# zzzxxxttt/SimpleDepthEstimation

Hardware: AMD Instinct MI355X
Metric: training images/sec at 192x640 bs=12/GPU (higher is better)
Workload: dtype bf16; 1 GPU; Supervised ResNet-50 (BASELINE configs[1]), bf16 storage / fp32 accumulate, bs=12/GPU, 192x640, fwd+bwd+optimizer, random-init weights; global_batch=12, parallelism=dp1, hip_graph=True, allreduce_overlap=False

## Files before the change

### include/sde_hip.h

```cpp
#ifndef SDE_HIP_H
#define SDE_HIP_H
#include <stddef.h>
#include <stdint.h>

#ifdef __cplusplus
extern "C" {
#endif

typedef void* sde_stream_t;

#define SDE_MAX_CTX 4
#define SDE_F32 0
#define SDE_BF16 1
#define SDE_F16 2

#define SDE_REDUCE_ROWS 32

#define SDE_RESIZE_BILINEAR_AC 0
#define SDE_RESIZE_NEAREST 1

const char* sde_last_error(void);
int sde_version(void);

int sde_mark_time(uint64_t* slot, sde_stream_t stream);
// ... 105 lines not shown
size_t sde_conv_fwd_ws_bytes(const sde_conv_desc* d, int ldy);
int sde_conv_fwd_ws(const sde_conv_desc* d, const void* w_packed, const float* bias, int act, void* y, int Cout, int ldy, float* stats, void* ws,
                    size_t ws_bytes, sde_stream_t stream);
int sde_conv_dgrad_bnbwd_rows(const sde_conv_desc* d, int Cout, int ldy);
int sde_conv_dgrad_bnbwd(const sde_conv_desc* d, const void* w_packed, void* gm, int Cout, int ldy, const void* bn_y, const float* bnp, float* part,
                         sde_stream_t stream);
int sde_conv_dgrad_bnbwd_res_rows(const sde_conv_desc* d, int Cout, int ldy);
int sde_conv_dgrad_bnbwd_res(const sde_conv_desc* d, const void* w_packed, void* gm, int Cout, int ldy, const void* bn_y, const float* bnp, float* part,
                             const void* res_grad, const void* bn_out, sde_stream_t stream);
int sde_conv_fwd_tiles_m(const sde_conv_desc* d, int ldy);
int sde_conv_fwd_variant(const sde_conv_desc* d, int ldy);
int sde_conv_set_halo_min_blocks(int min_blocks);
#define SDE_OPT_PGEMM 1
#define SDE_OPT_PGEMM_DEPTH 2
#define SDE_OPT_PGEMM_3X3 3
#define SDE_OPT_PGEMM_TILE 4
#define SDE_OPT_SPLITK 5
#define SDE_OPT_WGRAD_BLOCKS 6
#define SDE_OPT_WGRAD_HALO 7
#define SDE_OPT_CONV_SMALL 8
#define SDE_OPT_WGRAD_DMA 9
#define SDE_OPT_BNBWD_FUSE 10
#define SDE_OPT_CU_RESERVE 11
int sde_conv_set_option(int key, int value);

#define SDE_WGRAD_FOLD_ROWS 16
int sde_conv_wgrad_splits(const sde_conv_desc* d, int Cout);
int sde_conv_wgrad(const sde_conv_desc* d, const void* dy, int Cout, int ldd, int Cin_real, float* slab, int splits, float* dw, int accumulate,
                   sde_stream_t stream);

int sde_conv_wgrad_partial(const sde_conv_desc* d, const void* dy, int Cout, int ldd, float* slab, int splits, sde_stream_t stream);
typedef struct sde_wreduce_item {
    const float* slab;
    float* dw;
    int32_t rows , Cout, KHW, Cin_pad, Cin_real;
    int32_t accumulate;
} sde_wreduce_item;
#define SDE_WREDUCE_ACCUMULATE 1
#define SDE_WREDUCE_OHWI 2
int sde_wgrad_reduce_batched(const sde_wreduce_item* items, int n, sde_stream_t stream);

int sde_prep_input(const float* img, const float* mean, const float* std_, int B, int C, int H, int W, int Cpad, int flip, int dtype, void* out,
                   sde_stream_t stream);

int sde_bn_finalize(const float* part, int tiles, int C, long count, const float* gamma, const float* beta, float* running_mean, float* running_var,
                    float momentum, float eps, float* bnp, sde_stream_t stream);
// ... 145 lines not shown
```

### simpledepthestimation_amd/csrc/conv.hip

```cpp
#include <type_traits>

#include "common.h"
#include "sde_hip.h"
#include "conv_common.h"

namespace {
using namespace sdeconv;

template <int I> using IC = std::integral_constant<int, I>;

typedef __attribute__((ext_vector_type(4))) float f32x4;
typedef __attribute__((ext_vector_type(8))) __bf16 bf16x8;
typedef __attribute__((ext_vector_type(4))) short s16x4;
typedef __attribute__((ext_vector_type(8))) short s16x8;

template <typename T> struct VecOf;
template <> struct VecOf<float> { static constexpr int V = 4; };
template <> struct VecOf<bf16_t> { static constexpr int V = 8; };
template <> struct VecOf<half_t> { static constexpr int V = 8; };

template <typename T>
__device__ __forceinline__ uint4 gather16(const Gather& g, int n, int ih, int iw, int ci) {
    uint4 z = {0u, 0u, 0u, 0u};
    if (g.reflect) { ih = reflect1(ih, g.IH); iw = reflect1(iw, g.IW); }
// ... 1274 lines not shown
    if (d->src_mode == SDE_SRC_UPCAT) {
        if (d->IH != 2 * d->H0 || d->IW != 2 * d->W0 || (d->C1 > 0 && !d->x1)) { sde_set_error("%s: upcat shape mismatch", who); return SDE_ERR_ARG; }
    } else if (d->src_mode == SDE_SRC_PLAIN) {
        if (d->IH != d->H0 || d->IW != d->W0 || d->C1 != 0) { sde_set_error("%s: plain source shape mismatch", who); return SDE_ERR_ARG; }
    } else if (d->src_mode == SDE_SRC_ZEROINS) {
        if (d->IH > 2 * d->H0 || d->IW > 2 * d->W0 || d->IH < 2 * d->H0 - 1 || d->IW < 2 * d->W0 - 1 || d->C1 != 0) { sde_set_error("%s: zero-insert shape mismatch", who); return SDE_ERR_ARG; }
    } else { sde_set_error("%s: bad src_mode %d", who, d->src_mode); return SDE_ERR_ARG; }
    if (d->reflect && (d->pad >= d->IH || d->pad >= d->IW || d->pad > 1)) { sde_set_error("%s: reflection pad must be 1 and < size", who); return SDE_ERR_ARG; }
    const int oh_max = (d->OH - 1) * d->stride - d->pad + d->KH - 1, ow_max = (d->OW - 1) * d->stride - d->pad + d->KW - 1;
    if (d->reflect && (oh_max > d->IH || ow_max > d->IW)) { sde_set_error("%s: output extent exceeds reflected input", who); return SDE_ERR_ARG; }
    g.x0 = d->x0; g.x1 = d->x1; g.C0 = d->C0; g.C1 = d->C1; g.Cin = d->C0 + d->C1; g.H0 = d->H0; g.W0 = d->W0; g.IH = d->IH; g.IW = d->IW;
    g.mode = d->src_mode; g.KH = d->KH; g.KW = d->KW; g.stride = d->stride; g.pad = d->pad; g.reflect = d->reflect;
    g.Bn = d->Bn; g.OH = d->OH; g.OW = d->OW; g.M = d->Bn * d->OH * d->OW; g.Ktot = d->KH * d->KW * g.Cin;
    if ((long)d->Bn * d->OH * d->OW > 0x7fffffffL) { sde_set_error("%s: too many output pixels", who); return SDE_ERR_ARG; }
    return SDE_OK;
}

}

namespace sdeconv {
bool pgemm_applicable(const Gather& g, int dtype, int ldy);
bool pgemm_bnbwd_ok(const Gather& g, int dtype, int ldy, int Cout, int depth);
int pgemm_tile(const Gather& g, int ldy);
int pgemm_run(const IGemmP& p, int dtype, int depth, hipStream_t s);
int pgemm_stats_rows(const Gather& g, int ldy, int depth, bool bnbwd = false);
bool chalo_applicable(const Gather& g, int dtype, int ldy);
int chalo_run(const IGemmP& p, int dtype, hipStream_t s);
bool wgrad_dma_applicable(const Gather& g, int dtype, int Cout, int ldd);
int wgrad_dma_run(const Gather& g, int dtype, const void* dy, int Cout, int ldd, float* slab, int splits, int rows_per_split, hipStream_t s);
bool whalo_applicable(const Gather& g, int dtype, int Cout, int ldd);
int whalo_splits(const Gather& g, int Cout);
int whalo_run(const Gather& g, int dtype, const void* dy, int Cout, int ldd, float* slab, int splits, hipStream_t s);
extern int g_pgemm_force_tile;
}
namespace {
int g_use_pgemm = 1;
int g_pgemm_depth = 3;
int g_pgemm_3x3 = 0;
int g_splitk = 1;
long g_wgrad_blocks = 256;
bool use_pgemm(const Gather& g, int dtype, int ldy) {
    if (!g_use_pgemm || !pgemm_applicable(g, dtype, ldy)) return false;
    return g_pgemm_3x3 || !use_halo(g, dtype, ldy);
}
}

extern "C" {

static int pick_ksplit(const Gather& g, int dtype, int ldy) {
    const bool pg = use_pgemm(g, dtype, ldy);
    if (!g_splitk || ldy % 4) return 1;
    if (pg ? (pgemm_tile(g, ldy) != 64064 || g.mode == SDE_SRC_ZEROINS) : (use_halo(g, dtype, ldy) || pick_tile(g.M, ldy, g.Ktot) != 64064)) return 1;
    const long tiles = (long)sde_cdiv(g.M, 64) * sde_cdiv(ldy, 64);
    const int nk = sde_cdiv(g.Ktot, SDE_IS16(dtype) ? 64 : 32);
    const long tmax = pg ? 256 : 384, target = pg ? 512 : 768;
    if (pg && tiles >= tmax && tiles < 2 * tmax && nk >= (g_splitk >= 2 ? g_splitk : 48)) return 2;
    if (tiles >= tmax || nk < 16) return 1;
    long S = sde_cdiv(target, tiles);
    if (S > 8) S = 8;
    if (S > nk / 8) S = nk / 8;
    return S < 2 ? 1 : (int)S;
}

int g_conv_small = 1;
static bool use_chalo(const Gather& g, int dtype, int ldy) { return g_conv_small && sdeconv::chalo_applicable(g, dtype, ldy); }

static int conv_fwd_impl(const sde_conv_desc* d, const void* w_packed, const float* bias, int act, void* y, int Cout, int ldy, float* stats,
                         float* ws, size_t ws_bytes, sde_stream_t stream) {
    SDE_CHECK_ARG(d && w_packed && y, "sde_conv_fwd: null pointer");
    IGemmP p;
    int rc = fill_gather(d, p.g, "sde_conv_fwd");
    if (rc) return rc;
    SDE_CHECK_ARG(Cout > 0 && ldy >= Cout, "sde_conv_fwd: bad Cout=%d ldy=%d", Cout, ldy);
    SDE_CHECK_ARG(act == SDE_ACT_NONE || act == SDE_ACT_ELU, "sde_conv_fwd: bad act %d", act);
    p.w = w_packed; p.bias = bias; p.y = y; p.stats = stats; p.Cout = Cout; p.ldy = ldy; p.act = act;
    p.ksplit = 1; p.ws = nullptr;
    p.no_kfull = 0;
    p.bn_y = nullptr; p.bnp = nullptr; p.bn_gb = nullptr; p.bn_out = nullptr;
    const int S = ws ? pick_ksplit(p.g, d->dtype, ldy) : 1;
    if (S > 1) {
        SDE_CHECK_ARG(ws_bytes >= (size_t)S * p.g.M * ldy * sizeof(float), "sde_conv_fwd_ws: workspace too small (%zu bytes)", ws_bytes);
        p.ksplit = S; p.ws = ws;
    }
    if (!stats && p.ksplit == 1 && use_chalo(p.g, d->dtype, ldy)) {
        sdeconv::chalo_run(p, d->dtype, (hipStream_t)stream);
    } else if (use_pgemm(p.g, d->dtype, ldy)) {
        SDE_CHECK_ARG((p.ksplit - 1) * sde_cdiv(p.g.Ktot / 64, p.ksplit) < p.g.Ktot / 64, "sde_conv_fwd: empty K split");
        SDE_CHECK_ARG(p.ksplit == 1 || sdeconv::pgemm_stats_rows(p.g, ldy, g_pgemm_depth) == sde_cdiv(p.g.M, 64), "sde_conv_fwd: split-K layer with per-workgroup statistics");
        sdeconv::pgemm_run(p, d->dtype, g_pgemm_depth, (hipStream_t)stream);
    } else if (use_halo(p.g, d->dtype, ldy)) {
        if (d->dtype == SDE_BF16) dispatch_halo<bf16_t>(p, (hipStream_t)stream); else dispatch_halo<half_t>(p, (hipStream_t)stream);
    } else if (d->dtype == SDE_BF16) dispatch_igemm<bf16_t>(p, (hipStream_t)stream);
    else if (d->dtype == SDE_F16) dispatch_igemm<half_t>(p, (hipStream_t)stream);
    else dispatch_igemm<float>(p, (hipStream_t)stream);
    SDE_CHECK_LAUNCH("sde_conv_fwd");
    if (S > 1) {
        const unsigned nb = (unsigned)(sde_cdiv(p.g.M, 64) * sde_cdiv(ldy, 64));
        if (d->dtype == SDE_BF16) hipLaunchKernelGGL(splitk_finish_kernel<bf16_t>, dim3(nb), dim3(256), 0, (hipStream_t)stream, ws, S, p.g.M, ldy, Cout, bias, act, (bf16_t*)y, stats);
        else if (d->dtype == SDE_F16) hipLaunchKernelGGL(splitk_finish_kernel<half_t>, dim3(nb), dim3(256), 0, (hipStream_t)stream, ws, S, p.g.M, ldy, Cout, bias, act, (half_t*)y, stats);
        else hipLaunchKernelGGL(splitk_finish_kernel<float>, dim3(nb), dim3(256), 0, (hipStream_t)stream, ws, S, p.g.M, ldy, Cout, bias, act, (float*)y, stats);
        SDE_CHECK_LAUNCH("sde_conv_fwd/splitk_finish");
    }
    return SDE_OK;
}

int sde_conv_fwd(const sde_conv_desc* d, const void* w_packed, const float* bias, int act, void* y, int Cout, int ldy, float* stats,
                 sde_stream_t stream) {
    return conv_fwd_impl(d, w_packed, bias, act, y, Cout, ldy, stats, nullptr, 0, stream);
}

size_t sde_conv_fwd_ws_bytes(const sde_conv_desc* d, int ldy) {
    Gather g;
    if (!d || fill_gather(d, g, "sde_conv_fwd_ws_bytes") != SDE_OK) return 0;
    const int S = pick_ksplit(g, d->dtype, ldy);
    return S > 1 ? (size_t)S * g.M * ldy * sizeof(float) : 0;
}

int sde_conv_fwd_ws(const sde_conv_desc* d, const void* w_packed, const float* bias, int act, void* y, int Cout, int ldy, float* stats, void* ws,
                    size_t ws_bytes, sde_stream_t stream) {
    return conv_fwd_impl(d, w_packed, bias, act, y, Cout, ldy, stats, (float*)ws, ws_bytes, stream);
}

static int gather_of(const sde_conv_desc* d, Gather& g) { return fill_gather(d, g, "sde_conv_fwd_tiles_m"); }

int g_bnbwd_fuse = 1;

static int bnbwd_kind(const Gather& g, int dtype, int ldy, int Cout) {
    if (!g_bnbwd_fuse || !SDE_IS16(dtype) || ldy != Cout || Cout % 64 || g.mode != SDE_SRC_PLAIN || g.stride != 1 || g.reflect) return 0;
    if (pick_ksplit(g, dtype, ldy) != 1) return 0;
    if (use_chalo(g, dtype, ldy)) return 0;
    if (use_pgemm(g, dtype, ldy)) return sdeconv::pgemm_bnbwd_ok(g, dtype, ldy, Cout, g_pgemm_depth) ? 1 : 0;
    if (use_halo(g, dtype, ldy)) return halo_bn(g, ldy) == 64 ? 2 : 0;
    return 0;
}

int sde_conv_dgrad_bnbwd_rows(const sde_conv_desc* d, int Cout, int ldy) {
    Gather g;
    if (!d || fill_gather(d, g, "sde_conv_dgrad_bnbwd_rows") != SDE_OK) return 0;
// ... 208 lines not shown
    const size_t total = for_dgrad ? (size_t)Cin_pad * KH * KW * Cout_pad : (size_t)Cout_pad * KH * KW * Cin_pad;
    const int nb = (int)((total + 255) / 256 > 4096 ? 4096 : (total + 255) / 256);
    if (for_dgrad) {
        if (dtype == SDE_BF16) hipLaunchKernelGGL(pack_w_dgrad_kernel<bf16_t>, dim3(nb), dim3(256), 0, s, w, (bf16_t*)out, Cout, Cin, KH, KW, Cout_pad, Cin_pad);
        else if (dtype == SDE_F16) hipLaunchKernelGGL(pack_w_dgrad_kernel<half_t>, dim3(nb), dim3(256), 0, s, w, (half_t*)out, Cout, Cin, KH, KW, Cout_pad, Cin_pad);
        else hipLaunchKernelGGL(pack_w_dgrad_kernel<float>, dim3(nb), dim3(256), 0, s, w, (float*)out, Cout, Cin, KH, KW, Cout_pad, Cin_pad);
    } else {
        if (dtype == SDE_BF16) hipLaunchKernelGGL(pack_w_fwd_kernel<bf16_t>, dim3(nb), dim3(256), 0, s, w, (bf16_t*)out, Cout, Cin, KH, KW, Cin_pad, Cout_pad);
        else if (dtype == SDE_F16) hipLaunchKernelGGL(pack_w_fwd_kernel<half_t>, dim3(nb), dim3(256), 0, s, w, (half_t*)out, Cout, Cin, KH, KW, Cin_pad, Cout_pad);
        else hipLaunchKernelGGL(pack_w_fwd_kernel<float>, dim3(nb), dim3(256), 0, s, w, (float*)out, Cout, Cin, KH, KW, Cin_pad, Cout_pad);
    }
    SDE_CHECK_LAUNCH("sde_pack_weight");
    return SDE_OK;
}

int sde_conv_set_option(int key, int value) {
    if (key == SDE_OPT_WGRAD_BLOCKS) {
        SDE_CHECK_ARG(value >= 1 && value <= 65536, "sde_conv_set_option: bad workgroup target %d", value);
        const int old = (int)g_wgrad_blocks;
        g_wgrad_blocks = value;
        return old;
    }
    int* slot = key == SDE_OPT_PGEMM ? &g_use_pgemm : key == SDE_OPT_PGEMM_DEPTH ? &g_pgemm_depth : key == SDE_OPT_PGEMM_3X3 ? &g_pgemm_3x3 :
                key == SDE_OPT_PGEMM_TILE ? &sdeconv::g_pgemm_force_tile : key == SDE_OPT_SPLITK ? &g_splitk : key == SDE_OPT_WGRAD_HALO ? &g_wgrad_halo : key == SDE_OPT_CONV_SMALL ? &g_conv_small : key == SDE_OPT_WGRAD_DMA ? &g_wgrad_dma : key == SDE_OPT_BNBWD_FUSE ? &g_bnbwd_fuse : key == SDE_OPT_CU_RESERVE ? &sdeconv::g_cu_reserve : nullptr;
    SDE_CHECK_ARG(slot, "sde_conv_set_option: unknown key %d", key);
    SDE_CHECK_ARG(key != SDE_OPT_CU_RESERVE || (value >= 0 && value <= 128 && value % 8 == 0), "sde_conv_set_option: CU reserve must be a multiple of 8 in [0, 128], got %d", value);
    SDE_CHECK_ARG(key != SDE_OPT_PGEMM_DEPTH || value == 3 || value == 4, "sde_conv_set_option: ring depth must be 3 or 4");
    SDE_CHECK_ARG(key != SDE_OPT_PGEMM_TILE || value == 0 || value == 64064 || value == 128064 || value == 128128, "sde_conv_set_option: bad tile %d", value);
    const int old = *slot;
    *slot = value;
    return old;
}

int sde_conv_set_halo_min_blocks(int min_blocks) {
    const int old = g_halo_min_blocks;
    g_halo_min_blocks = min_blocks;
    return old;
}

int sde_pack_item_blocks(int Cout_pad, int Cin_pad, int KH, int KW) {
    if (Cout_pad <= 0 || Cin_pad <= 0 || KH <= 0 || KW <= 0 || (long)PACK_CO * 8 * KH * KW + PACK_CO > PACK_LDS_FLOATS) return -1;
    return sde_cdiv(Cout_pad, PACK_CO) * sde_cdiv(Cin_pad, pack_ci(KH * KW));
}

int sde_pack_weights_batched(const sde_pack_item* items_dev, int n, long total_blocks, int dtype, sde_stream_t stream) {
    SDE_CHECK_ARG(items_dev && n > 0 && total_blocks > 0 && total_blocks < 0x7fffffffL, "sde_pack_weights_batched: bad argument");
    SDE_CHECK_ARG(SDE_DTYPE_OK(dtype), "sde_pack_weights_batched: bad dtype");
// ... 9 lines not shown
```

### simpledepthestimation_amd/csrc/conv_common.h

```cpp
#pragma once
#include "common.h"
#include "sde_hip.h"

namespace sdeconv {

extern int g_cu_reserve;
int sde_persistent_cus();

__device__ __forceinline__ int reflect1(int i, int n) {
    if (i < 0) i = -i;
    if (i >= n) i = 2 * (n - 1) - i;
    return i;
}

struct Gather {
    const void* x0; const void* x1;
    int C0, C1, Cin;
    int H0, W0;
    int IH, IW;
    int mode;
    int KH, KW, stride, pad, reflect;
    int Bn, OH, OW, M;
    int Ktot;
};
// ... 15 lines not shown
    int ksplit;
    float* ws;
    int no_kfull;
    const void* bn_y;
    const float* bnp;
    const void* bn_gb;
    const void* bn_out;
};


typedef __attribute__((ext_vector_type(4))) unsigned int u32x4;
constexpr unsigned kOOB = 0x80000000u;

__device__ __forceinline__ __amdgpu_buffer_rsrc_t make_rsrc(const void* p, long bytes) {
    return __builtin_amdgcn_make_buffer_rsrc(const_cast<void*>(p), 0, (int)(bytes > 0x7fffffffL ? 0x7fffffffL : bytes), 0x00020000);
}
__device__ __forceinline__ uint4 buf_load16s(__amdgpu_buffer_rsrc_t r, unsigned voff, unsigned soff) {
    return __builtin_bit_cast(uint4, __builtin_amdgcn_raw_buffer_load_b128(r, voff, soff, 0));
}
__device__ __forceinline__ uint4 buf_load16(__amdgpu_buffer_rsrc_t r, unsigned off) {
    return __builtin_bit_cast(uint4, __builtin_amdgcn_raw_buffer_load_b128(r, off, 0, 0));
}

constexpr int SRC_RUNTIME = -1, SRC_PLAIN_ZERO = 0, SRC_PLAIN_REFLECT = 1, SRC_UPCAT_REFLECT = 2, SRC_ZEROINS_ZERO = 3, SRC_1X1 = 4;

}
```

### simpledepthestimation_amd/csrc/pgemm.hip

```cpp
#include "conv_common.h"

namespace sdeconv {

typedef __attribute__((ext_vector_type(8))) __bf16 pg_bf16x8;
typedef __attribute__((ext_vector_type(16))) float pg_f32x16;
typedef __attribute__((ext_vector_type(4))) float pg_f32x4;
typedef __attribute__((ext_vector_type(2))) float pg_f32x2;
template <int V> struct PgIC { static constexpr int value = V; };
typedef __attribute__((address_space(3))) void pg_lds_void;

constexpr int PG_THREADS = 256;
constexpr int PG_STAGE_K_BYTES = 128;

template <int N> __device__ __forceinline__ void pg_wait_vmcnt() { asm volatile("s_waitcnt vmcnt(%0)" ::"n"(N) : "memory"); }

__device__ __forceinline__ void pg_dma16(__amdgpu_buffer_rsrc_t r, unsigned char* lds, unsigned voff, unsigned soff) {
    __builtin_amdgcn_raw_ptr_buffer_load_lds(r, (pg_lds_void*)lds, 16, voff, soff, 0, 0);
}
__device__ __forceinline__ void pg_dma4(__amdgpu_buffer_rsrc_t r, unsigned char* lds, unsigned voff) {
    __builtin_amdgcn_raw_ptr_buffer_load_lds(r, (pg_lds_void*)lds, 4, voff, 0, 0, 0);
}

template <typename T16> struct PgType;
template <> struct PgType<bf16_t> {
// ... 23 lines not shown
    }
};

typedef __attribute__((ext_vector_type(2))) unsigned pg_u32x2;
__device__ __forceinline__ unsigned pg_lds_addr(const void* p) { return (unsigned)(unsigned long)(__attribute__((address_space(3))) const void*)p; }
__device__ __forceinline__ void pg_lds_store8(unsigned addr, unsigned a, unsigned b) {
    pg_u32x2 v = {a, b};
    asm volatile("ds_write_b64 %0, %1" ::"v"(addr), "v"(v) : "memory");
}

__device__ __forceinline__ void pg_lds_store16(unsigned addr, float a, float b, float c, float d) {
    const pg_f32x4 v = {a, b, c, d};
    asm volatile("ds_write_b128 %0, %1" ::"v"(addr), "v"(v) : "memory");
}

struct PGemmP {
    IGemmP p;
    int tiles_n, tiles_mn, total;
    int nk_total, nk_per;
    int cls_end[4];
    int zero_siblings;
    int stats_acc;
    int fast, tm_step;
};

struct PGWork {
    int tile_m, tile_n, split, s_begin, nk;
    int cls;
};

struct PGClass {
    int a, b, ih0, iw0, IHc, IWc, nta, ntb, M;
};
__host__ __device__ inline PGClass pg_class(const Gather& g, int c) {
    PGClass k;
    k.a = c >> 1; k.b = c & 1;
    k.ih0 = (k.a + g.pad) & 1; k.iw0 = (k.b + g.pad) & 1;
    k.IHc = g.OH > k.ih0 ? (g.OH - k.ih0 + 1) / 2 : 0; k.IWc = g.OW > k.iw0 ? (g.OW - k.iw0 + 1) / 2 : 0;
    k.nta = g.KH > k.a ? (g.KH - k.a + 1) / 2 : 0; k.ntb = g.KW > k.b ? (g.KW - k.b + 1) / 2 : 0;
    k.M = g.Bn * k.IHc * k.IWc;
    return k;
}

template <int BM, int BN, int SRC>
__device__ __forceinline__ PGWork pg_work(const PGemmP& q, int w) {
    PGWork r;
// ... 8 lines not shown
        r.nk = k.nta * k.ntb * (q.p.g.C0 / 64);
        return r;
    }
    r.cls = 0;
    r.split = logical / q.tiles_mn;
    const int rem = logical - r.split * q.tiles_mn;
    r.tile_m = rem / q.tiles_n;
    r.tile_n = rem - r.tile_m * q.tiles_n;
    r.s_begin = r.split * q.nk_per;
    const int e = r.s_begin + q.nk_per;
    r.nk = (e < q.nk_total ? e : q.nk_total) - r.s_begin;
    if (r.nk < 0) r.nk = 0;
    return r;
}

template <int BM, int BN, int SRC>
__device__ __forceinline__ PGWork pg_next(const PGemmP& q, const PGWork& wk, int w_next) {
    if (q.fast) { PGWork r = wk; r.tile_m += q.tm_step; return r; }
    return pg_work<BM, BN, SRC>(q, w_next);
}

__device__ __forceinline__ void pg_lds_store4(unsigned addr, unsigned a) { asm volatile("ds_write_b32 %0, %1" ::"v"(addr), "v"(a) : "memory"); }

template <typename T16, int BM, int BN, int SRC, int D, bool BNB = false, int NW = 4, int WGM = 2>
__global__ void __launch_bounds__(64 * NW) pgemm_kernel(const PGemmP q) {
    typedef typename PgType<T16>::frag frag_t;
    constexpr int PG_THREADS = 64 * NW;
    constexpr int WGN = NW / WGM;
    constexpr int WTM = BM / WGM, WTN = BN / WGN;
    constexpr int FM = WTM / 32, FN = WTN / 32;
    constexpr int XP = BM / (8 * NW), WP = BN / (8 * NW);
    static_assert(BM % (8 * NW) == 0 && BN % (8 * NW) == 0 && WTM % 32 == 0 && WTN % 32 == 0, "tile / wave grid");
    constexpr int L = XP + WP;
    constexpr int STAGE_BYTES = (BM + BN) * PG_STAGE_K_BYTES;
    constexpr int BIAS_BYTES = BN * 4;
    constexpr int SLOT_BYTES = STAGE_BYTES;
    constexpr int BIAS_BASE = D * STAGE_BYTES;
    constexpr int EN = BN > 64 ? 64 : BN, NCH = BN / EN;
    constexpr int CST = EN * 2 + 16;
    constexpr int ST = PG_THREADS > 256 ? 256 : PG_THREADS;
    static_assert(BM * CST + (ST / (EN / 2)) * EN * 8 <= STAGE_BYTES, "the output staging tile and the statistics scratch must fit into one ring slot");
    static_assert(D >= 3 && (D - 2) * L <= 60, "ring depth");
    extern __shared__ __attribute__((aligned(16))) unsigned char smem[];

    const IGemmP& p = q.p;
    const Gather& g = p.g;
    const int tid = threadIdx.x, lane = tid & 63;
// ... 211 lines not shown
#pragma unroll
            for (int kk = 0; kk < 4; ++kk)
#pragma unroll
                for (int j = 0; j < FN; ++j)
#pragma unroll
                    for (int i = 0; i < FM; ++i) acc[j][i] = PgType<T16>::mma(wf[kk][j], xf[kk][i], acc[j][i]);
            ++consumed;
        }

        if (p.ksplit > 1) {
            float* wsp = p.ws + (size_t)wk.split * g.M * p.ldy;
#pragma unroll
            for (int i = 0; i < FM; ++i) {
                const int m = m0 + wm * WTM + i * 32 + l31;
#pragma unroll
                for (int j = 0; j < FN; ++j)
#pragma unroll
                    for (int gq = 0; gq < 4; ++gq) {
                        const int n = n0 + wn * WTN + j * 32 + 8 * gq + 4 * lh;
                        if (m < g.M && n < p.ldy)
                            *reinterpret_cast<float4*>(wsp + (size_t)m * p.ldy + n) =
                                make_float4(acc[j][i][4 * gq], acc[j][i][4 * gq + 1], acc[j][i][4 * gq + 2], acc[j][i][4 * gq + 3]);
                    }
            }
            ++c_item;
            continue;
        }
        unsigned char* sC = smem + ((consumed - 1) % D) * SLOT_BYTES;
        const unsigned sC_a = pg_lds_addr(sC);
        const float* sbias = reinterpret_cast<const float*>(smem + BIAS_BASE + (c_item % D) * BIAS_BYTES);
#pragma unroll
        for (int ch = 0; ch < NCH; ++ch) {
            __builtin_amdgcn_s_barrier();
            auto stage_values = [&](auto ELU, auto RAGGED) {
#pragma unroll
                for (int j = 0; j < FN; ++j) {
                    if ((wn * WTN + j * 32) / EN != ch) continue;
#pragma unroll
                    for (int i = 0; i < FM; ++i) {
                        const int row = wm * WTM + i * 32 + l31;
#pragma unroll
                        for (int gq = 0; gq < 4; ++gq) {
                            const int nt = wn * WTN + j * 32 + 8 * gq + 4 * lh;
                            const pg_f32x4 b4 = *reinterpret_cast<const pg_f32x4*>(sbias + nt);
                            float v[4];
#pragma unroll
// ... 209 lines not shown
            float a = 0.f, b = 0.f;
#pragma unroll
            for (int z = 0; z < PARTS; ++z) { a += red[((ch * PARTS + z) * EN + c) * 2]; b += red[((ch * PARTS + z) * EN + c) * 2 + 1]; }
            p.stats[((size_t)row * p.Cout + st_n0 + id) * 2 + 0] = a;
            p.stats[((size_t)row * p.Cout + st_n0 + id) * 2 + 1] = b;
        }
    }
}

static int pg_grid_max(int BM, int BN, int D) {
    const int lds = D * ((BM + BN) * PG_STAGE_K_BYTES + BN * 4);
    const int per_cu = (160 * 1024) / lds;
#ifndef PG_MAX_PER_CU
#define PG_MAX_PER_CU 4
#endif
    return sde_persistent_cus() * (per_cu < 1 ? 1 : (per_cu > PG_MAX_PER_CU ? PG_MAX_PER_CU : per_cu));
}

static bool pg_stats_acc(int tiles_n, int tiles_mn, int ksplit, int src, int BM, int BN, int D) {
    const int grid = pg_grid_max(BM, BN, D);
    return ksplit == 1 && src != SRC_ZEROINS_ZERO && tiles_mn > grid && (grid >> 3) % tiles_n == 0;
}

template <typename T16, int BM, int BN, int SRC, int D, bool BNB = false, int NW = 4, int WGM = 2>
static int pg_launch(const PGemmP& q, hipStream_t s) {
    constexpr int lds = D * ((BM + BN) * PG_STAGE_K_BYTES + BN * 4);
    static bool attr_done = false;
    if (!attr_done) {
        (void)hipFuncSetAttribute(reinterpret_cast<const void*>(&pgemm_kernel<T16, BM, BN, SRC, D, BNB, NW, WGM>), hipFuncAttributeMaxDynamicSharedMemorySize, lds);
        attr_done = true;
    }
    int grid = pg_grid_max(BM, BN, D);
    if (grid > q.total) grid = q.total;
    PGemmP qq = q;
    qq.fast = (q.p.ksplit == 1 && SRC != SRC_ZEROINS_ZERO && grid % 8 == 0 && (grid >> 3) % q.tiles_n == 0) ? 1 : 0;
    qq.tm_step = qq.fast ? (grid >> 3) / q.tiles_n : 0;
    hipLaunchKernelGGL((pgemm_kernel<T16, BM, BN, SRC, D, BNB, NW, WGM>), dim3(grid), dim3(64 * NW), lds, s, qq);
    return 0;
}

template <typename T16, int BM, int BN, int D, int NW = 4, int WGM = 2>
static int pg_dispatch_src(const PGemmP& q, int src, hipStream_t s) {
    switch (src) {
        case SRC_1X1: return pg_launch<T16, BM, BN, SRC_1X1, D, false, NW, WGM>(q, s);
        case SRC_PLAIN_ZERO: return pg_launch<T16, BM, BN, SRC_PLAIN_ZERO, D, false, NW, WGM>(q, s);
        case SRC_PLAIN_REFLECT: return pg_launch<T16, BM, BN, SRC_PLAIN_REFLECT, D, false, NW, WGM>(q, s);
        case SRC_ZEROINS_ZERO: return pg_launch<T16, BM, BN, SRC_ZEROINS_ZERO, D, false, NW, WGM>(q, s);
        default: return pg_launch<T16, BM, BN, SRC_UPCAT_REFLECT, D, false, NW, WGM>(q, s);
    }
}

bool pgemm_applicable(const Gather& g, int dtype, int ldy) {
    if (!SDE_IS16(dtype)) return false;
    if (g.Cin % 64 || g.C0 % 64 || (g.mode == SDE_SRC_UPCAT && !g.reflect)) return false;
    if (g.mode == SDE_SRC_ZEROINS) {
        if (g.reflect || g.stride != 1 || g.KH != g.KW || g.pad < 0) return false;
        if (g.KH == 1 && g.pad != 0) return false;
    }
    if (ldy % 8) return false;
    if ((long)g.Bn * g.IH * g.IW * (g.C0 > g.C1 ? g.C0 : g.C1) * 2L >= 0x7fffffffL) return false;
    return true;
}

int pgemm_src_kind(const Gather& g) {
    if (g.mode == SDE_SRC_UPCAT) return SRC_UPCAT_REFLECT;
    if (g.mode == SDE_SRC_ZEROINS) return SRC_ZEROINS_ZERO;
    if (g.KH == 1 && g.KW == 1 && g.pad == 0 && !g.reflect) return SRC_1X1;
    return g.reflect ? SRC_PLAIN_REFLECT : SRC_PLAIN_ZERO;
}

int g_cu_reserve = 0;
int sde_persistent_cus() {
    static int cus = 0;
    if (!cus) {
        int dev = 0, n = 0;
        if (hipGetDevice(&dev) != hipSuccess || hipDeviceGetAttribute(&n, hipDeviceAttributeMultiprocessorCount, dev) != hipSuccess || n < 8) n = 256;
        cus = n;
    }
    const int left = cus - g_cu_reserve;
    return left < 8 ? 8 : left;
}
int g_pgemm_force_tile = 0;
int pgemm_tile(const Gather& g, int ldy) {
    (void)g; (void)ldy;
    return g_pgemm_force_tile ? g_pgemm_force_tile : 64064;
}

static int pg_depth(int tile, int depth) { return tile != 64064 || depth == 3 ? 3 : 4; }

bool pgemm_bnbwd_ok(const Gather& g, int dtype, int ldy, int Cout, int depth) {
    if (!pgemm_applicable(g, dtype, ldy) || depth != 3 || (g_pgemm_force_tile && g_pgemm_force_tile != 64064)) return false;
    const int src = pgemm_src_kind(g);
    return (src == SRC_1X1 || src == SRC_PLAIN_ZERO) && g.stride == 1 && Cout % 64 == 0 && ldy == Cout;
}

template <typename T16>
static int pgemm_run_t(const PGemmP& q, int tile, int src, int depth, hipStream_t s) {
    if (q.p.bn_y) return src == SRC_1X1 ? pg_launch<T16, 64, 64, SRC_1X1, 3, true>(q, s) : pg_launch<T16, 64, 64, SRC_PLAIN_ZERO, 3, true>(q, s);
    if (tile == 128128) return pg_dispatch_src<T16, 128, 128, 3, 8, 2>(q, src, s);
    if (tile == 128064) return pg_dispatch_src<T16, 128, 64, 3, 8, 4>(q, src, s);
    return depth == 3 ? pg_dispatch_src<T16, 64, 64, 3>(q, src, s) : pg_dispatch_src<T16, 64, 64, 4>(q, src, s);
}

int pgemm_run(const IGemmP& p, int dtype, int depth, hipStream_t s) {
    PGemmP q;
    q.p = p;
    const int tile = p.bn_y ? 64064 : pgemm_tile(p.g, p.ldy);
    const int BM = tile / 1000, BN = tile % 1000;
    q.tiles_n = sde_cdiv(p.ldy, BN);
    q.tiles_mn = sde_cdiv(p.g.M, BM) * q.tiles_n;
    q.total = q.tiles_mn * p.ksplit;
    q.nk_total = p.g.Ktot / 64;
    q.nk_per = sde_cdiv(q.nk_total, p.ksplit);
    const int src = pgemm_src_kind(p.g);
    q.zero_siblings = 0;
    q.stats_acc = p.stats && pg_stats_acc(q.tiles_n, q.tiles_mn, p.ksplit, src, BM, BN, pg_depth(tile, depth)) ? 1 : 0;
    for (int c = 0; c < 4; ++c) q.cls_end[c] = 0;
    if (src == SRC_ZEROINS_ZERO) {
        int end = 0;
        for (int c = 0; c < 4; ++c) {
            const PGClass k = pg_class(p.g, c);
            if (k.nta > 0 && k.ntb > 0) end += sde_cdiv(k.M, BM) * q.tiles_n;
            q.cls_end[c] = end;
        }
        q.total = end;
        q.zero_siblings = (p.g.KH == 1 && p.g.KW == 1) ? 1 : 0;
        if (q.total == 0) return 0;
    }
    return dtype == SDE_F16 ? pgemm_run_t<half_t>(q, tile, src, depth, s) : pgemm_run_t<bf16_t>(q, tile, src, depth, s);
// ... 13 lines not shown
```

### simpledepthestimation_amd/hip/nn.py

```python
import contextlib
import ctypes
import functools
import os
import weakref
from collections import namedtuple
from ctypes import POINTER, Structure, c_float, c_int, c_int32, c_long, c_void_p

import torch

from . import lib as L

SRC_PLAIN, SRC_UPCAT, SRC_ZEROINS = 0, 1, 2
REDUCE_ROWS = 32
ACT_NONE, ACT_ELU, ACT_RELU = 0, 1, 2


class ConvDesc(Structure):
    _fields_ = [("x0", c_void_p), ("x1", c_void_p), ("dtype", c_int32), ("C0", c_int32), ("C1", c_int32), ("H0", c_int32), ("W0", c_int32),
                ("IH", c_int32), ("IW", c_int32), ("src_mode", c_int32), ("KH", c_int32), ("KW", c_int32), ("stride", c_int32), ("pad", c_int32),
                ("reflect", c_int32), ("Bn", c_int32), ("OH", c_int32), ("OW", c_int32)]


_P, _I, _F, _LG = c_void_p, c_int, c_float, c_long
L.register_protos({
# ... 36 lines not shown
    "sde_refl_fold": ([_P, _I, _I, _I, _I, _I, _I, _I, _P, _P, _P], c_int),
    "sde_depth_head_fwd": ([_P, _I, _I, _I, _I, _F, _F, _I, _I, _P, _P], c_int),
    "sde_depth_head_bwd": ([_P, _P, _I, _I, _I, _I, _F, _F, _I, _I, _P, _P], c_int),
    "sde_gn_relu_fwd": ([_P, _P, _P, _I, _I, _I, _I, _F, _I, _I, _P, _P, _P, _P], c_int),
    "sde_gn_relu_bwd": ([_P, _P, _P, _P, _P, _I, _I, _I, _I, _I, _I, _P, _P, _P, _P, _I, _P, _P], c_int),
    "sde_gn_relu_res_fwd": ([_P, _P, _P, _P, _I, _I, _I, _I, _F, _I, _I, _P, _P, _P, _P], c_int),
    "sde_gn_relu_res_bwd": ([_P, _P, _P, _P, _P, _P, _I, _I, _I, _I, _I, _I, _P, _P, _P, _P, _I, _P, _P], c_int),
    "sde_space_to_depth": ([_P, _I, _I, _I, _I, _I, _P, _P], c_int),
    "sde_depth_to_space": ([_P, _I, _I, _I, _I, _I, _P, _P], c_int),
    "sde_concat_fwd": ([_P, _P, _P, _I, _I, _I, _I, _I, _I, _I, _I, _P, _P], c_int),
    "sde_concat_bwd": ([_P, _I, _I, _I, _I, _I, _I, _I, _I, _P, _P, _P, _P], c_int),
    "sde_inv_depth_head_fwd": ([_P, _I, _I, _I, _I, _F, _F, _F, _I, _I, _P, _P, _P], c_int),
    "sde_inv_depth_head_bwd": ([_P, _P, _P, _I, _I, _I, _I, _F, _F, _F, _I, _I, _P, _P], c_int),
    "sde_conv3d_fwd": ([_P, _P, _P, _I, _I, _I, _I, _I, _P, _P], c_int),
    "sde_conv3d_dgrad": ([_P, _P, _I, _I, _I, _I, _I, _P, _P], c_int),
    "sde_conv3d_wgrad_num_blocks": ([_I, _I, _I, _I, _I], c_int),
    "sde_conv3d_wgrad": ([_P, _P, _I, _I, _I, _I, _I, _P, _P, _P, _I, _P], c_int),
    "sde_adam_step": ([_P, _P, _P, _P, _LG, _P, _P], c_int),
    "sde_grad_check": ([_P, _LG, _P, _P], c_int),
    "sde_loss_scale_update": ([_P, _F, _F, _I, _P], c_int),
})


OPT_PGEMM, OPT_PGEMM_DEPTH, OPT_PGEMM_3X3, OPT_PGEMM_TILE, OPT_SPLITK, OPT_WGRAD_BLOCKS, OPT_WGRAD_HALO, OPT_CONV_SMALL, OPT_WGRAD_DMA, OPT_BNBWD_FUSE, OPT_CU_RESERVE = 1, 2, 3, 4, 5, 6, 7, 8, 9, 10, 11


def set_option(key, value):
    old = L.lib().sde_conv_set_option(int(key), int(value))
    if old < 0:
        raise L.SdeHipError(f"sde_conv_set_option({key}, {value}) failed: {L.lib().sde_last_error().decode()}")
    return old


def dtype_code(dt):
    if dt == torch.float32:
        return L.F32
    if dt == torch.bfloat16:
        return L.BF16
    if dt == torch.float16:
        return L.F16
    raise L.SdeHipError(f"unsupported activation dtype {dt}")


def vec_of(dt):
    return 4 if dt == torch.float32 else 8


# ... 946 lines not shown
```

Measured before the change: 1881 images/s.

## Fuse split-K reduction into pgemm via last-arriver atomic tile counters

For split-K forward convolutions on the 64x64 pgemm path, each workgroup now bumps a per-tile counter in a workspace header with a token-tagged CAS. The last split to finish a tile sums the fp32 partial slabs and applies bias, ELU, the bf16 store and the BN statistics in place, so the separate splitk_finish_kernel launch is skipped. This removes one kernel launch per split-K layer and its tail, in exchange for atomics, fences, a serial reduction inside the GEMM kernel and a 4KB workspace header.

New measurement: 1826 images/s. -2.9%, worse.

```diff
diff --git a/include/sde_hip.h b/include/sde_hip.h
--- a/include/sde_hip.h
+++ b/include/sde_hip.h
@@ -151,6 +151,7 @@
 #define SDE_OPT_WGRAD_DMA 9
 #define SDE_OPT_BNBWD_FUSE 10
 #define SDE_OPT_CU_RESERVE 11
+#define SDE_OPT_SPLITK_COMBINE 12
 int sde_conv_set_option(int key, int value);
 
 #define SDE_WGRAD_FOLD_ROWS 16
diff --git a/simpledepthestimation_amd/csrc/conv.hip b/simpledepthestimation_amd/csrc/conv.hip
--- a/simpledepthestimation_amd/csrc/conv.hip
+++ b/simpledepthestimation_amd/csrc/conv.hip
@@ -1,3 +1,4 @@
+#include <atomic>
 #include <type_traits>
 
 #include "common.h"
@@ -1320,7 +1321,8 @@
 bool pgemm_applicable(const Gather& g, int dtype, int ldy);
 bool pgemm_bnbwd_ok(const Gather& g, int dtype, int ldy, int Cout, int depth);
 int pgemm_tile(const Gather& g, int ldy);
-int pgemm_run(const IGemmP& p, int dtype, int depth, hipStream_t s);
+int pgemm_run(const IGemmP& p, int dtype, int depth, hipStream_t s, unsigned* cnt = nullptr, unsigned token = 0);
+bool pgemm_combine_ok(const Gather& g, int ldy, int ksplit);
 int pgemm_stats_rows(const Gather& g, int ldy, int depth, bool bnbwd = false);
 bool chalo_applicable(const Gather& g, int dtype, int ldy);
 int chalo_run(const IGemmP& p, int dtype, hipStream_t s);
@@ -1336,6 +1338,7 @@
 int g_pgemm_depth = 3;
 int g_pgemm_3x3 = 0;
 int g_splitk = 1;
+int g_splitk_combine = 1;
 long g_wgrad_blocks = 256;
 bool use_pgemm(const Gather& g, int dtype, int ldy) {
     if (!g_use_pgemm || !pgemm_applicable(g, dtype, ldy)) return false;
@@ -1360,6 +1363,8 @@
     return S < 2 ? 1 : (int)S;
 }
 
+static size_t splitk_ws_bytes(int S, int M, int ldy) { return (size_t)sdeconv::PGEMM_WS_HEADER_BYTES + (size_t)S * M * ldy * sizeof(float); }
+
 int g_conv_small = 1;
 static bool use_chalo(const Gather& g, int dtype, int ldy) { return g_conv_small && sdeconv::chalo_applicable(g, dtype, ldy); }
 
@@ -1376,23 +1381,31 @@
     p.no_kfull = 0;
     p.bn_y = nullptr; p.bnp = nullptr; p.bn_gb = nullptr; p.bn_out = nullptr;
     const int S = ws ? pick_ksplit(p.g, d->dtype, ldy) : 1;
+    bool combine = false;
+    unsigned token = 0;
     if (S > 1) {
-        SDE_CHECK_ARG(ws_bytes >= (size_t)S * p.g.M * ldy * sizeof(float), "sde_conv_fwd_ws: workspace too small (%zu bytes)", ws_bytes);
-        p.ksplit = S; p.ws = ws;
+        SDE_CHECK_ARG(ws_bytes >= splitk_ws_bytes(S, p.g.M, ldy), "sde_conv_fwd_ws: workspace too small (%zu bytes)", ws_bytes);
+        p.ksplit = S; p.ws = reinterpret_cast<float*>(reinterpret_cast<char*>(ws) + sdeconv::PGEMM_WS_HEADER_BYTES);
+        combine = g_splitk_combine && use_pgemm(p.g, d->dtype, ldy) && sdeconv::pgemm_combine_ok(p.g, ldy, S);
+        if (combine) {
+            static std::atomic<unsigned> next_token{0};
+            do token = ((next_token.fetch_add(1, std::memory_order_relaxed) + 1u) * 0x9E3779B1u) >> 4; while (token == 0);
+        }
     }
     if (!stats && p.ksplit == 1 && use_chalo(p.g, d->dtype, ldy)) {
         sdeconv::chalo_run(p, d->dtype, (hipStream_t)stream);
     } else if (use_pgemm(p.g, d->dtype, ldy)) {
         SDE_CHECK_ARG((p.ksplit - 1) * sde_cdiv(p.g.Ktot / 64, p.ksplit) < p.g.Ktot / 64, "sde_conv_fwd: empty K split");
         SDE_CHECK_ARG(p.ksplit == 1 || sdeconv::pgemm_stats_rows(p.g, ldy, g_pgemm_depth) == sde_cdiv(p.g.M, 64), "sde_conv_fwd: split-K layer with per-workgroup statistics");
-        sdeconv::pgemm_run(p, d->dtype, g_pgemm_depth, (hipStream_t)stream);
+        sdeconv::pgemm_run(p, d->dtype, g_pgemm_depth, (hipStream_t)stream, combine ? reinterpret_cast<unsigned*>(ws) : nullptr, token);
     } else if (use_halo(p.g, d->dtype, ldy)) {
         if (d->dtype == SDE_BF16) dispatch_halo<bf16_t>(p, (hipStream_t)stream); else dispatch_halo<half_t>(p, (hipStream_t)stream);
     } else if (d->dtype == SDE_BF16) dispatch_igemm<bf16_t>(p, (hipStream_t)stream);
     else if (d->dtype == SDE_F16) dispatch_igemm<half_t>(p, (hipStream_t)stream);
     else dispatch_igemm<float>(p, (hipStream_t)stream);
     SDE_CHECK_LAUNCH("sde_conv_fwd");
-    if (S > 1) {
+    if (S > 1 && !combine) {
+        const float* ws = p.ws;
         const unsigned nb = (unsigned)(sde_cdiv(p.g.M, 64) * sde_cdiv(ldy, 64));
         if (d->dtype == SDE_BF16) hipLaunchKernelGGL(splitk_finish_kernel<bf16_t>, dim3(nb), dim3(256), 0, (hipStream_t)stream, ws, S, p.g.M, ldy, Cout, bias, act, (bf16_t*)y, stats);
         else if (d->dtype == SDE_F16) hipLaunchKernelGGL(splitk_finish_kernel<half_t>, dim3(nb), dim3(256), 0, (hipStream_t)stream, ws, S, p.g.M, ldy, Cout, bias, act, (half_t*)y, stats);
@@ -1411,7 +1424,7 @@
     Gather g;
     if (!d || fill_gather(d, g, "sde_conv_fwd_ws_bytes") != SDE_OK) return 0;
     const int S = pick_ksplit(g, d->dtype, ldy);
-    return S > 1 ? (size_t)S * g.M * ldy * sizeof(float) : 0;
+    return S > 1 ? splitk_ws_bytes(S, g.M, ldy) : 0;
 }
 
 int sde_conv_fwd_ws(const sde_conv_desc* d, const void* w_packed, const float* bias, int act, void* y, int Cout, int ldy, float* stats, void* ws,
@@ -1666,7 +1679,7 @@
         return old;
     }
     int* slot = key == SDE_OPT_PGEMM ? &g_use_pgemm : key == SDE_OPT_PGEMM_DEPTH ? &g_pgemm_depth : key == SDE_OPT_PGEMM_3X3 ? &g_pgemm_3x3 :
-                key == SDE_OPT_PGEMM_TILE ? &sdeconv::g_pgemm_force_tile : key == SDE_OPT_SPLITK ? &g_splitk : key == SDE_OPT_WGRAD_HALO ? &g_wgrad_halo : key == SDE_OPT_CONV_SMALL ? &g_conv_small : key == SDE_OPT_WGRAD_DMA ? &g_wgrad_dma : key == SDE_OPT_BNBWD_FUSE ? &g_bnbwd_fuse : key == SDE_OPT_CU_RESERVE ? &sdeconv::g_cu_reserve : nullptr;
+                key == SDE_OPT_PGEMM_TILE ? &sdeconv::g_pgemm_force_tile : key == SDE_OPT_SPLITK ? &g_splitk : key == SDE_OPT_SPLITK_COMBINE ? &g_splitk_combine : key == SDE_OPT_WGRAD_HALO ? &g_wgrad_halo : key == SDE_OPT_CONV_SMALL ? &g_conv_small : key == SDE_OPT_WGRAD_DMA ? &g_wgrad_dma : key == SDE_OPT_BNBWD_FUSE ? &g_bnbwd_fuse : key == SDE_OPT_CU_RESERVE ? &sdeconv::g_cu_reserve : nullptr;
     SDE_CHECK_ARG(slot, "sde_conv_set_option: unknown key %d", key);
     SDE_CHECK_ARG(key != SDE_OPT_CU_RESERVE || (value >= 0 && value <= 128 && value % 8 == 0), "sde_conv_set_option: CU reserve must be a multiple of 8 in [0, 128], got %d", value);
     SDE_CHECK_ARG(key != SDE_OPT_PGEMM_DEPTH || value == 3 || value == 4, "sde_conv_set_option: ring depth must be 3 or 4");
diff --git a/simpledepthestimation_amd/csrc/conv_common.h b/simpledepthestimation_amd/csrc/conv_common.h
--- a/simpledepthestimation_amd/csrc/conv_common.h
+++ b/simpledepthestimation_amd/csrc/conv_common.h
@@ -61,6 +61,8 @@
     return __builtin_bit_cast(uint4, __builtin_amdgcn_raw_buffer_load_b128(r, off, 0, 0));
 }
 
+constexpr int PGEMM_WS_HEADER_BYTES = 4096;
+
 constexpr int SRC_RUNTIME = -1, SRC_PLAIN_ZERO = 0, SRC_PLAIN_REFLECT = 1, SRC_UPCAT_REFLECT = 2, SRC_ZEROINS_ZERO = 3, SRC_1X1 = 4;
 
 }
diff --git a/simpledepthestimation_amd/csrc/pgemm.hip b/simpledepthestimation_amd/csrc/pgemm.hip
--- a/simpledepthestimation_amd/csrc/pgemm.hip
+++ b/simpledepthestimation_amd/csrc/pgemm.hip
@@ -69,6 +69,8 @@
     int zero_siblings;
     int stats_acc;
     int fast, tm_step;
+    unsigned* cnt;
+    unsigned token;
 };
 
 struct PGWork {
@@ -123,7 +125,34 @@
 
 __device__ __forceinline__ void pg_lds_store4(unsigned addr, unsigned a) { asm volatile("ds_write_b32 %0, %1" ::"v"(addr), "v"(a) : "memory"); }
 
-template <typename T16, int BM, int BN, int SRC, int D, bool BNB = false, int NW = 4, int WGM = 2>
+typedef __attribute__((address_space(1))) unsigned pg_gu32;
+__device__ __forceinline__ unsigned pg_cas_agent(unsigned* p, unsigned expect, unsigned desired) {
+    const pg_u32x2 d = {desired, expect};
+    unsigned old;
+    asm volatile("global_atomic_cmpswap %0, %1, %2, off sc0\n\ts_waitcnt vmcnt(0)" : "=&v"(old) : "v"(p), "v"(d) : "memory");
+    return old;
+}
+__device__ __forceinline__ void pg_load_8x16_4x4(pg_f32x4 (&v)[8], const float* const (&a)[8], float (&b)[4], const float* const (&ba)[4]) {
+    asm volatile(
+        "global_load_dwordx4 %0, %12, off\n\tglobal_load_dwordx4 %1, %13, off\n\tglobal_load_dwordx4 %2, %14, off\n\tglobal_load_dwordx4 %3, %15, off\n\t"
+        "global_load_dwordx4 %4, %16, off\n\tglobal_load_dwordx4 %5, %17, off\n\tglobal_load_dwordx4 %6, %18, off\n\tglobal_load_dwordx4 %7, %19, off\n\t"
+        "global_load_dword %8, %20, off\n\tglobal_load_dword %9, %21, off\n\tglobal_load_dword %10, %22, off\n\tglobal_load_dword %11, %23, off\n\t"
+        "s_waitcnt vmcnt(0)"
+        : "=&v"(v[0]), "=&v"(v[1]), "=&v"(v[2]), "=&v"(v[3]), "=&v"(v[4]), "=&v"(v[5]), "=&v"(v[6]), "=&v"(v[7]), "=&v"(b[0]), "=&v"(b[1]), "=&v"(b[2]), "=&v"(b[3])
+        : "v"(a[0]), "v"(a[1]), "v"(a[2]), "v"(a[3]), "v"(a[4]), "v"(a[5]), "v"(a[6]), "v"(a[7]), "v"(ba[0]), "v"(ba[1]), "v"(ba[2]), "v"(ba[3])
+        : "memory");
+}
+__device__ __forceinline__ void pg_load_8x16(pg_f32x4 (&v)[8], const float* const (&a)[8]) {
+    asm volatile(
+        "global_load_dwordx4 %0, %8, off\n\tglobal_load_dwordx4 %1, %9, off\n\tglobal_load_dwordx4 %2, %10, off\n\tglobal_load_dwordx4 %3, %11, off\n\t"
+        "global_load_dwordx4 %4, %12, off\n\tglobal_load_dwordx4 %5, %13, off\n\tglobal_load_dwordx4 %6, %14, off\n\tglobal_load_dwordx4 %7, %15, off\n\t"
+        "s_waitcnt vmcnt(0)"
+        : "=&v"(v[0]), "=&v"(v[1]), "=&v"(v[2]), "=&v"(v[3]), "=&v"(v[4]), "=&v"(v[5]), "=&v"(v[6]), "=&v"(v[7])
+        : "v"(a[0]), "v"(a[1]), "v"(a[2]), "v"(a[3]), "v"(a[4]), "v"(a[5]), "v"(a[6]), "v"(a[7])
+        : "memory");
+}
+
+template <typename T16, int BM, int BN, int SRC, int D, bool BNB = false, int NW = 4, int WGM = 2, bool COMB = false>
 __global__ void __launch_bounds__(64 * NW) pgemm_kernel(const PGemmP q) {
     typedef typename PgType<T16>::frag frag_t;
     constexpr int PG_THREADS = 64 * NW;
@@ -381,6 +410,107 @@
                             *reinterpret_cast<float4*>(wsp + (size_t)m * p.ldy + n) =
                                 make_float4(acc[j][i][4 * gq], acc[j][i][4 * gq + 1], acc[j][i][4 * gq + 2], acc[j][i][4 * gq + 3]);
                     }
+            }
+            if constexpr (COMB) {
+                static_assert(BM == 64 && BN == 64 && NW == 4 && !BNB, "the reducer repeats splitk_finish_kernel's 64x64 / 256-thread mapping");
+                constexpr int FLAG_OFF = 16 * 64 * 2 * 4;
+                static_assert(FLAG_OFF + 16 <= STAGE_BYTES, "reducer scratch must fit into one ring slot");
+                unsigned char* sR = smem + ((consumed - 1) % D) * SLOT_BYTES;
+                const unsigned sR_a = pg_lds_addr(sR);
+                pg_wait_vmcnt<0>();
+                __builtin_amdgcn_s_barrier();
+                if (tid == 0) {
+                    __builtin_amdgcn_fence(__ATOMIC_RELEASE, "agent");
+                    pg_wait_vmcnt<0>();
+                    unsigned* word = q.cnt + wk.tile_m * q.tiles_n + wk.tile_n;
+                    unsigned expect = 0, desired;
+                    for (;;) {
+                        desired = (expect >> 4) == q.token ? expect + 1 : (q.token << 4 | 1u);
+                        const unsigned found = pg_cas_agent(word, expect, desired);
+                        if (found == expect) break;
+                        expect = found;
+                    }
+                    const unsigned last = (desired & 15u) == (unsigned)p.ksplit ? 1u : 0u;
+                    if (last) {
+                        __hip_atomic_store((pg_gu32*)word, 0u, __ATOMIC_RELAXED, __HIP_MEMORY_SCOPE_AGENT);
+                        __builtin_amdgcn_fence(__ATOMIC_ACQUIRE, "agent");
+                        pg_wait_vmcnt<0>();
+                    }
+                    pg_lds_store4(sR_a + FLAG_OFF, last);
+                }
+                asm volatile("s_waitcnt lgkmcnt(0)" ::: "memory");
+                __builtin_amdgcn_s_barrier();
+                if (*reinterpret_cast<const unsigned*>(sR + FLAG_OFF)) {
+                    const int S = p.ksplit;
+                    const int cq = tid & 15, rg = tid >> 4;
+                    const int c0 = n0 + cq * 4;
+                    const bool col_ok = c0 < p.ldy;
+                    const size_t slab = (size_t)g.M * p.ldy;
+                    const float* rowp[4];
+#pragma unroll
+                    for (int i = 0; i < 4; ++i) {
+                        const int m = m0 + rg + 16 * i;
+                        rowp[i] = p.ws + (size_t)(m < g.M ? m : m0) * p.ldy + (col_ok ? c0 : n0);
+                    }
+                    pg_f32x4 a[4], v[8];
+                    float bv[4];
+                    {
+                        const float* const ad[8] = {rowp[0], rowp[1], rowp[2], rowp[3], rowp[0] + slab, rowp[1] + slab, rowp[2] + slab, rowp[3] + slab};
+                        const float* const bd[4] = {p.bias && c0 + 0 < p.Cout ? p.bias + c0 + 0 : rowp[0], p.bias && c0 + 1 < p.Cout ? p.bias + c0 + 1 : rowp[0],
+                                                    p.bias && c0 + 2 < p.Cout ? p.bias + c0 + 2 : rowp[0], p.bias && c0 + 3 < p.Cout ? p.bias + c0 + 3 : rowp[0]};
+                        pg_load_8x16_4x4(v, ad, bv, bd);
+#pragma unroll
+                        for (int i = 0; i < 4; ++i) a[i] = v[i] + v[4 + i];
+                    }
+#pragma unroll 1
+                    for (int sp = 2; sp < S; sp += 2) {
+                        const size_t o0 = (size_t)sp * slab, o1 = (size_t)(sp + 1 < S ? sp + 1 : sp) * slab;
+                        const float* const ad[8] = {rowp[0] + o0, rowp[1] + o0, rowp[2] + o0, rowp[3] + o0, rowp[0] + o1, rowp[1] + o1, rowp[2] + o1, rowp[3] + o1};
+                        pg_load_8x16(v, ad);
+#pragma unroll
+                        for (int i = 0; i < 4; ++i) a[i] += v[i];
+                        if (sp + 1 < S) {
+#pragma unroll
+                            for (int i = 0; i < 4; ++i) a[i] += v[4 + i];
+                        }
+                    }
+                    float s1[4] = {0.f, 0.f, 0.f, 0.f}, s2[4] = {0.f, 0.f, 0.f, 0.f};
+                    if (col_ok) {
+#pragma unroll
+                        for (int i = 0; i < 4; ++i) {
+                            const int m = m0 + rg + 16 * i;
+                            if (m >= g.M) continue;
+                            T16 o[4];
+#pragma unroll
+                            for (int e = 0; e < 4; ++e) {
+                                float t = a[i][e];
+                                if (p.bias && c0 + e < p.Cout) t += bv[e];
+                                if (p.act == SDE_ACT_ELU) t = t > 0.f ? t : expm1f(t);
+                                if (c0 + e >= p.Cout) t = 0.f;
+                                o[e] = (T16)t;
+                                const float r = (float)o[e];
+                                s1[e] += r; s2[e] += r * r;
+                            }
+                            *reinterpret_cast<pg_u32x2*>((T16*)p.y + (size_t)m * p.ldy + c0) = *reinterpret_cast<const pg_u32x2*>(o);
+                        }
+                    }
+                    if (p.stats) {
+#pragma unroll
+                        for (int e = 0; e < 4; e += 2) pg_lds_store16(sR_a + (rg * 64 + cq * 4 + e) * 8, s1[e], s2[e], s1[e + 1], s2[e + 1]);
+                        asm volatile("s_waitcnt lgkmcnt(0)" ::: "memory");
+                        __builtin_amdgcn_s_barrier();
+                        if (tid < 64 && n0 + tid < p.Cout) {
+                            float sa = 0.f, sb = 0.f;
+#pragma unroll
+                            for (int z = 0; z < 16; ++z) {
+                                const pg_f32x2 t = *reinterpret_cast<const pg_f32x2*>(sR + ((z * 64 + tid) * 2) * 4);
+                                sa += t[0]; sb += t[1];
+                            }
+                            p.stats[((size_t)wk.tile_m * p.Cout + n0 + tid) * 2 + 0] = sa;
+                            p.stats[((size_t)wk.tile_m * p.Cout + n0 + tid) * 2 + 1] = sb;
+                        }
+                    }
+                }
             }
             ++c_item;
             continue;
@@ -636,12 +766,12 @@
     return ksplit == 1 && src != SRC_ZEROINS_ZERO && tiles_mn > grid && (grid >> 3) % tiles_n == 0;
 }
 
-template <typename T16, int BM, int BN, int SRC, int D, bool BNB = false, int NW = 4, int WGM = 2>
+template <typename T16, int BM, int BN, int SRC, int D, bool BNB = false, int NW = 4, int WGM = 2, bool COMB = false>
 static int pg_launch(const PGemmP& q, hipStream_t s) {
     constexpr int lds = D * ((BM + BN) * PG_STAGE_K_BYTES + BN * 4);
     static bool attr_done = false;
     if (!attr_done) {
-        (void)hipFuncSetAttribute(reinterpret_cast<const void*>(&pgemm_kernel<T16, BM, BN, SRC, D, BNB, NW, WGM>), hipFuncAttributeMaxDynamicSharedMemorySize, lds);
+        (void)hipFuncSetAttribute(reinterpret_cast<const void*>(&pgemm_kernel<T16, BM, BN, SRC, D, BNB, NW, WGM, COMB>), hipFuncAttributeMaxDynamicSharedMemorySize, lds);
         attr_done = true;
     }
     int grid = pg_grid_max(BM, BN, D);
@@ -649,7 +779,7 @@
     PGemmP qq = q;
     qq.fast = (q.p.ksplit == 1 && SRC != SRC_ZEROINS_ZERO && grid % 8 == 0 && (grid >> 3) % q.tiles_n == 0) ? 1 : 0;
     qq.tm_step = qq.fast ? (grid >> 3) / q.tiles_n : 0;
-    hipLaunchKernelGGL((pgemm_kernel<T16, BM, BN, SRC, D, BNB, NW, WGM>), dim3(grid), dim3(64 * NW), lds, s, qq);
+    hipLaunchKernelGGL((pgemm_kernel<T16, BM, BN, SRC, D, BNB, NW, WGM, COMB>), dim3(grid), dim3(64 * NW), lds, s, qq);
     return 0;
 }
 
@@ -664,6 +794,16 @@
     }
 }
 
+template <typename T16, int D>
+static int pg_dispatch_comb(const PGemmP& q, int src, hipStream_t s) {
+    switch (src) {
+        case SRC_1X1: return pg_launch<T16, 64, 64, SRC_1X1, D, false, 4, 2, true>(q, s);
+        case SRC_PLAIN_ZERO: return pg_launch<T16, 64, 64, SRC_PLAIN_ZERO, D, false, 4, 2, true>(q, s);
+        case SRC_PLAIN_REFLECT: return pg_launch<T16, 64, 64, SRC_PLAIN_REFLECT, D, false, 4, 2, true>(q, s);
+        default: return pg_launch<T16, 64, 64, SRC_UPCAT_REFLECT, D, false, 4, 2, true>(q, s);
+    }
+}
+
 bool pgemm_applicable(const Gather& g, int dtype, int ldy) {
     if (!SDE_IS16(dtype)) return false;
     if (g.Cin % 64 || g.C0 % 64 || (g.mode == SDE_SRC_UPCAT && !g.reflect)) return false;
@@ -700,6 +840,11 @@
     return g_pgemm_force_tile ? g_pgemm_force_tile : 64064;
 }
 
+bool pgemm_combine_ok(const Gather& g, int ldy, int ksplit) {
+    return ksplit > 1 && ksplit <= 15 && pgemm_tile(g, ldy) == 64064 && pgemm_src_kind(g) != SRC_ZEROINS_ZERO &&
+           (long)sde_cdiv(g.M, 64) * sde_cdiv(ldy, 64) <= PGEMM_WS_HEADER_BYTES / 4;
+}
+
 static int pg_depth(int tile, int depth) { return tile != 64064 || depth == 3 ? 3 : 4; }
 
 bool pgemm_bnbwd_ok(const Gather& g, int dtype, int ldy, int Cout, int depth) {
@@ -710,15 +855,17 @@
 
 template <typename T16>
 static int pgemm_run_t(const PGemmP& q, int tile, int src, int depth, hipStream_t s) {
+    if (q.cnt) return depth == 3 ? pg_dispatch_comb<T16, 3>(q, src, s) : pg_dispatch_comb<T16, 4>(q, src, s);
     if (q.p.bn_y) return src == SRC_1X1 ? pg_launch<T16, 64, 64, SRC_1X1, 3, true>(q, s) : pg_launch<T16, 64, 64, SRC_PLAIN_ZERO, 3, true>(q, s);
     if (tile == 128128) return pg_dispatch_src<T16, 128, 128, 3, 8, 2>(q, src, s);
     if (tile == 128064) return pg_dispatch_src<T16, 128, 64, 3, 8, 4>(q, src, s);
     return depth == 3 ? pg_dispatch_src<T16, 64, 64, 3>(q, src, s) : pg_dispatch_src<T16, 64, 64, 4>(q, src, s);
 }
 
-int pgemm_run(const IGemmP& p, int dtype, int depth, hipStream_t s) {
+int pgemm_run(const IGemmP& p, int dtype, int depth, hipStream_t s, unsigned* cnt, unsigned token) {
     PGemmP q;
     q.p = p;
+    q.cnt = cnt; q.token = token;
     const int tile = p.bn_y ? 64064 : pgemm_tile(p.g, p.ldy);
     const int BM = tile / 1000, BN = tile % 1000;
     q.tiles_n = sde_cdiv(p.ldy, BN);
diff --git a/simpledepthestimation_amd/hip/nn.py b/simpledepthestimation_amd/hip/nn.py
--- a/simpledepthestimation_amd/hip/nn.py
+++ b/simpledepthestimation_amd/hip/nn.py
@@ -82,7 +82,7 @@
 })
 
 
-OPT_PGEMM, OPT_PGEMM_DEPTH, OPT_PGEMM_3X3, OPT_PGEMM_TILE, OPT_SPLITK, OPT_WGRAD_BLOCKS, OPT_WGRAD_HALO, OPT_CONV_SMALL, OPT_WGRAD_DMA, OPT_BNBWD_FUSE, OPT_CU_RESERVE = 1, 2, 3, 4, 5, 6, 7, 8, 9, 10, 11
+OPT_PGEMM, OPT_PGEMM_DEPTH, OPT_PGEMM_3X3, OPT_PGEMM_TILE, OPT_SPLITK, OPT_WGRAD_BLOCKS, OPT_WGRAD_HALO, OPT_CONV_SMALL, OPT_WGRAD_DMA, OPT_BNBWD_FUSE, OPT_CU_RESERVE, OPT_SPLITK_COMBINE = 1, 2, 3, 4, 5, 6, 7, 8, 9, 10, 11, 12
 
 
 def set_option(key, value):
```
